# BrianPugh/tamp

Measured on AMD Instinct MI355X. Metric: input MB/s, 4KiB-chunk batch compress window=10 (bit-exact vs C ref), higher is better.
Workload: dtype u8

## Files before the change

### tamp_amd/csrc/tamp_common.hpp

```cpp
#pragma once
#include <hip/hip_runtime.h>
#include <stdint.h>

namespace tamp_amd {

constexpr int kWave = 64;
constexpr uint32_t kRing = 16;
constexpr uint32_t kPendMax = 256;
constexpr uint32_t kRleMax = 241;
constexpr uint32_t kRleWindowMax = 8;
constexpr uint32_t kExtExtraMax = 120;
constexpr int kSymRle = 12, kSymExt = 13, kSymFlush = 14;

enum : int8_t {
    kOk = 0,
    kOutputFull = 1,
    kInputExhausted = 2,
    kError = -1,
    kExcessBits = -2,
    kInvalidConf = -3,
    kOob = -4,
    kBadArgument = -21,
};

constexpr uint32_t kMaxDecodeIn = (1u << 29) - 1;
constexpr uint32_t kMaxDecodeCall = 1u << 28;

constexpr uint8_t kCodeTab[15] = {0x00, 0x03, 0x08, 0x0b, 0x14, 0x24, 0x26, 0x2b, 0x4b, 0x54, 0x94, 0x95, 0xaa, 0x27, 0xab};
constexpr uint8_t kNbitsTab[15] = {2, 3, 5, 5, 6, 7, 7, 7, 8, 8, 9, 9, 9, 7, 9};
constexpr uint64_t pack_bytes(const uint8_t* v, int first, int count) {
    uint64_t r = 0;
    for (int i = 0; i < count; i++) r |= (uint64_t)v[first + i] << (8 * i);
    return r;
}
constexpr uint64_t pack_nibbles(const uint8_t* v, int count) {
    uint64_t r = 0;
    for (int i = 0; i < count; i++) r |= (uint64_t)v[i] << (4 * i);
    return r;
}
constexpr uint64_t kCodeLo = pack_bytes(kCodeTab, 0, 8), kCodeHi = pack_bytes(kCodeTab, 8, 7);
constexpr uint64_t kNbitsPacked = pack_nibbles(kNbitsTab, 15);
static_assert(kCodeLo == 0x2b2624140b080300ull && kCodeHi == 0x00ab27aa9594544bull && kNbitsPacked == 0x979998877765532ull,
              "packed prefix code");
__device__ __forceinline__ uint32_t tok_code(uint32_t i) {
    return (uint32_t)((i < 8 ? kCodeLo >> (8 * i) : kCodeHi >> (8 * (i - 8))) & 0xFF);
}
__device__ __forceinline__ uint32_t tok_nbits(uint32_t i) { return (uint32_t)(kNbitsPacked >> (4 * i)) & 15; }

__host__ __device__ constexpr uint32_t align_up(uint32_t x, uint32_t a) { return (x + a - 1) & ~(a - 1); }

constexpr uint32_t kPackedMaxWbits = 14;
constexpr uint32_t max_code_nbits() {
    uint32_t m = 0;
    for (int i = 0; i < 15; i++) m = kNbitsTab[i] > m ? kNbitsTab[i] : m;
    return m;
}
constexpr uint32_t max_u32(uint32_t a, uint32_t b) { return a > b ? a : b; }
constexpr uint32_t kMaxTokenBits =
    max_u32(max_u32(1 + 8, max_code_nbits() + 15),
            max_u32(kNbitsTab[kSymRle] + max_code_nbits() - 1 + 4, kNbitsTab[kSymExt] + max_code_nbits() - 1 + 3 + kPackedMaxWbits));
static_assert(kMaxTokenBits <= 32, "a token is placed as one 32-bit value: at most two words of the bit buffer");

__host__ __device__ __forceinline__ void token_words(uint32_t v, uint32_t nb, uint32_t bitpos, uint32_t* wi, uint32_t* w_hi,
                                                     uint32_t* w_lo) {
    const uint32_t ph = bitpos & 31u;
    const uint64_t x = (uint64_t)v << (64u - ph - nb);
    *wi = bitpos >> 5;
    *w_hi = __builtin_bswap32((uint32_t)(x >> 32));
    *w_lo = __builtin_bswap32((uint32_t)x);
}

constexpr uint32_t kDictOffAlign = 16;
__host__ __device__ constexpr bool dict_off_aligned(uint64_t off) { return (off & (kDictOffAlign - 1)) == 0; }
__host__ __device__ constexpr bool dict_off_in_bounds(uint64_t off, uint32_t W, uint64_t len) { return off <= len && W <= len - off; }

__host__ __device__ constexpr int min_pattern_size(int window, int literal) {
    return 2 + (window > 10 + 2 * (literal - 5));
}

struct __attribute__((packed, aligned(1))) LdsU128 { uint32_t x, y, z, w; };

__device__ __forceinline__ uint32_t lds_u32_unaligned(const uint8_t* base, uint32_t off) {
    const uint32_t* w = reinterpret_cast<const uint32_t*>(base + (off & ~3u));
    return __builtin_amdgcn_alignbyte(w[1], w[0], off & 3u);
}

#if defined(__HIP_DEVICE_COMPILE__) && !defined(__GFX9__)
#error "tamp_amd device code is written for gfx9-family wave64 targets (gfx950); its DPP scans have no gfx10+ form"
#endif
template <class Op>
__device__ __forceinline__ uint32_t wave_scan_incl(uint32_t x, uint32_t identity, Op op) {
    x = op(x, (uint32_t)__builtin_amdgcn_update_dpp((int)identity, (int)x, 0x111, 0xF, 0xF, false));
    x = op(x, (uint32_t)__builtin_amdgcn_update_dpp((int)identity, (int)x, 0x112, 0xF, 0xF, false));
    x = op(x, (uint32_t)__builtin_amdgcn_update_dpp((int)identity, (int)x, 0x114, 0xF, 0xF, false));
    x = op(x, (uint32_t)__builtin_amdgcn_update_dpp((int)identity, (int)x, 0x118, 0xF, 0xF, false));
    x = op(x, (uint32_t)__builtin_amdgcn_update_dpp((int)identity, (int)x, 0x142, 0xA, 0xF, false));
    x = op(x, (uint32_t)__builtin_amdgcn_update_dpp((int)identity, (int)x, 0x143, 0xC, 0xF, false));
    return x;
}
__device__ __forceinline__ uint32_t wave_scan_add(uint32_t x) {
    return wave_scan_incl(x, 0u, [](uint32_t a, uint32_t b) { return a + b; });
}
__device__ __forceinline__ uint32_t wave_scan_max(uint32_t x) {
    return wave_scan_incl(x, 0u, [](uint32_t a, uint32_t b) { return a > b ? a : b; });
}

__device__ __forceinline__ uint32_t wave_max_u32(uint32_t v) {
#pragma unroll
    for (int off = 32; off > 0; off >>= 1) {
        uint32_t o = (uint32_t)__shfl_xor((int)v, off);
        v = o > v ? o : v;
    }
    return v;
}

}
```

### tamp_amd/csrc/tamp_compress_kernel.hpp

```cpp
#pragma once
#include "tamp_common.hpp"

namespace tamp_amd {

constexpr uint32_t kHashBits = 11;
constexpr uint32_t kHashBuckets = 1u << kHashBits;
constexpr uint32_t kRemBits = 16 - kHashBits;
constexpr uint32_t kRunCap = 128;
constexpr int kPrioScan = 0, kPrioShort = 2, kPrioWalk = 3;
constexpr uint32_t kDeferMin = 24;
constexpr uint32_t kDeferred = 0x1Fu;
constexpr uint32_t kLongRun = 8;
constexpr uint32_t kSlowCap = 128;
constexpr uint32_t kHb1024 = 10;

struct CompressArgs {
    const uint8_t* in;
    const uint64_t* in_off;
    const uint32_t* in_len;
    uint8_t* out;
    const uint64_t* out_off;
    const uint32_t* out_cap;
    uint32_t* out_len;
    int8_t* status;
// ... 525 lines not shown
                    }
                }
                ext_count = len;
                ext_pos = idx;
                rd += len;
                return kStepOk;
            }
            put((tok_code(len - minp) << wbits) | idx, tok_nbits(len - minp) + wbits);
        }
        const uint32_t rd0 = rd;
        rd += len;
        append(len, wr + len == rd, [&](uint32_t i) { return uni(ebuf[W + rd0 + i]); });
        return kStepOk;
    }
};

constexpr uint32_t kWgPerCu = 8, kLeanPerCu = 6, kLazyPerCu = 5;
constexpr uint32_t kBrkShift = 0, kBrkMin = 512;
constexpr uint32_t kAlignMin = 256;
enum : uint32_t { kActDone = 1, kActRebase = 2, kActContinue = 3 };
enum : uint8_t { kSegResume = 1, kSegSave = 2, kSegFlushToken = 4, kSegPartial = 8 };
enum : uint32_t {
    kSlotWindowPos = 0,
    kSlotToken = 2,
    kSlotRle = 3,
    kSlotExtCount = 4,
    kSlotNbits = 5,
    kSlotExtPos = 6,
    kSlotParsed = 9,
    kSlotBits = 16,
};
constexpr uint32_t kSegStateExtra = 24;
enum : uint32_t { cAct = 0, cShift = 1, cP0 = 2, cPending = 3, cWp = 4, cNtok = 5, cExcess = 6, cBlk = 7, cWave = 8, cNruns = 12, cQuad = 13, cNext = 14, cCut = 15, cCutThr = 16 };

#ifdef TAMP_PROF
#define TAMP_PROF_ONLY(...) __VA_ARGS__
#define TAMP_DBG(bit) ((a.dbg & (bit)) != 0)
#define TAMP_REPEAT(bit) for (uint32_t _rep = 0; _rep < (TAMP_DBG(bit) ? 2u : 1u); _rep++)
#define TAMP_SECOND (_rep != 0)
#define TAMP_FINE(v) do { unsigned long long _n = __builtin_readcyclecounter(); v += _n - fc; fc = _n; } while (0)
#define TAMP_PROF_MARK(i)                                     \
    do {                                                      \
        __syncthreads();                                      \
        unsigned long long _n = __builtin_readcyclecounter(); \
        pt[i] += _n - pc;                                     \
        pc = _n;                                              \
        if (TAMP_DBG(8u << (i))) return;                      \
    } while (0)
#else
#define TAMP_PROF_ONLY(...)
#define TAMP_DBG(bit) false
#define TAMP_REPEAT(bit)
#define TAMP_SECOND false
#define TAMP_FINE(v) do { } while (0)
#define TAMP_PROF_MARK(i) do { } while (0)
#endif

template <class T>
__device__ __forceinline__ T* as_global(T* p) {
    return (T*)(__attribute__((address_space(1))) T*)reinterpret_cast<uintptr_t>(p);
}

enum : uint32_t { kFixNone = 0, kFixExt = 1, kFixV1 = 2 };
constexpr uint32_t kFixWbits = 10, kFixBlk = 1024, kFixLbits = 8, kFixThreads = 256;
constexpr CompressLds kLdsFixed(1u << kFixWbits, kFixBlk, true, false, true, kHb1024);
static_assert(kLdsFixed.total == 19616 && kLdsFixed.tokcap == 1376 && kLdsFixed.obuf_words == 516,
              "the fixed builds' LDS layout is the generic build's for window 2^10, block 1,024, 1,024 buckets");
template <bool FX>
__device__ __forceinline__ uint8_t* lds_base() {
    if constexpr (FX) {
        __shared__ __attribute__((aligned(16))) uint8_t smem_fx[kLdsFixed.total];
        return smem_fx;
    } else {
        extern __shared__ __attribute__((aligned(16))) uint8_t smem[];
        return smem;
    }
}
template <bool PACKED, bool LAZY, bool RUNS, uint32_t WSCAN, uint32_t HB, bool LOOP, bool BLOCKM, uint32_t FIX, bool DICTS = false>
__device__ __forceinline__ void compress_streams(CompressArgs a_k) {
    static_assert(!DICTS || FIX == kFixNone, "table calls take the generic builds");
    static_assert(!BLOCKM || (LOOP && PACKED && !LAZY), "block mode: a persistent build of the default parse");
    constexpr bool FX = FIX != kFixNone;
    constexpr bool kFoldSort = FX, kOrTail = FX;
    static_assert(!FX || (PACKED && !LAZY && RUNS && WSCAN == (1u << kFixWbits) && HB == kHb1024 && LOOP && !BLOCKM),
                  "fixed geometry: the run-aware persistent build of the 2^10 window");
    static_assert(HB >= 9 && HB <= 11, "entry payload: 16 - HB bigram bits + 8 bits of the third byte + the rest of the fourth");
    constexpr uint32_t kRem = 16 - HB, kBuckets = 1u << HB;
    constexpr bool kEntV2 = PACKED && !LAZY;
    constexpr uint32_t kPB = WSCAN == 1024 ? 12u : 16u, kLB = 32u - kRem - kPB;
    static_assert(!kEntV2 || kLB >= 9, "the third byte and at least one bit of the fourth");
    static_assert(!(RUNS && LAZY), "the run list serves the default parse only");
    uint8_t* const smem = lds_base<FX>();
    typedef __attribute__((address_space(3))) volatile uint32_t LdsWord;
    constexpr uint32_t kNoClaim = 0xFFFFFFFFu;
    LdsWord* const claim = (LdsWord*)smem;
    if constexpr (LOOP) {
        if (threadIdx.x == 0) {
            const uint32_t nx = atomicAdd(a_k.work_counter, a_k.claim);
            claim[2] = nx, claim[0] = nx + 1, claim[1] = nx + a_k.claim, claim[3] = kNoClaim;
        }
        __syncthreads();
    }
    typedef const __attribute__((address_space(4))) uint32_t* KernArgs;
    struct ArgWords { uint32_t w[sizeof(CompressArgs) / 4]; };
    static_assert(sizeof(ArgWords) == sizeof(CompressArgs), "whole dwords");
    KernArgs ap = (KernArgs)__builtin_amdgcn_kernarg_segment_ptr();
    uint32_t wave_k = Walk::uni(threadIdx.x >> 6);
    for (;;) {
        ArgWords aw;
        if constexpr (LOOP) {
            asm volatile("" : "+s"(ap));
#pragma unroll
            for (uint32_t i = 0; i < (DICTS ? (uint32_t)(sizeof(CompressArgs) / 4) : kPlainArgWords); i++) aw.w[i] = ap[i];
        }
        CompressArgs a_l = __builtin_bit_cast(CompressArgs, aw);
        if constexpr (LOOP) {
            a_l.in = as_global(a_l.in), a_l.in_off = as_global(a_l.in_off), a_l.in_len = as_global(a_l.in_len);
            a_l.out = as_global(a_l.out), a_l.out_off = as_global(a_l.out_off), a_l.out_cap = as_global(a_l.out_cap);
            a_l.out_len = as_global(a_l.out_len), a_l.status = as_global(a_l.status), a_l.dict = as_global(a_l.dict);
            a_l.state = as_global(a_l.state), a_l.work_counter = as_global(a_l.work_counter), a_l.prof = as_global(a_l.prof);
            a_l.blk_table = as_global(a_l.blk_table), a_l.blk_info = as_global(a_l.blk_info);
            a_l.blk_len = as_global(a_l.blk_len), a_l.blk_idx = as_global(a_l.blk_idx);
            if constexpr (DICTS) a_l.dict_off = as_global(a_l.dict_off);
        }
        const CompressArgs& a = LOOP ? a_l : a_k;
        const uint32_t a_wbits = FX ? kFixWbits : a.wbits, a_blk = FX ? kFixBlk : a.blk;
        const uint32_t W = 1u << a_wbits, mask = W - 1;
        constexpr bool lazy = LAZY;
        const CompressLds L = FX ? kLdsFixed : CompressLds(W, a_blk, PACKED, lazy, RUNS, HB == 9 ? kHashBits : HB);
        uint8_t* const ebuf = smem + L.ebuf;
        uint16_t* const cnt16 = reinterpret_cast<uint16_t*>(smem + L.cnt);
        uint32_t* const cntw = reinterpret_cast<uint32_t*>(smem + L.cnt);
        uint32_t* const ent = reinterpret_cast<uint32_t*>(smem + L.ent);
        uint16_t* const ent16 = reinterpret_cast<uint16_t*>(smem + L.ent);
        uint16_t* const toklist = reinterpret_cast<uint16_t*>(smem + L.ent);
        uint16_t* const jump16 = reinterpret_cast<uint16_t*>(smem + L.ent + L.jump);
        uint8_t* const count8 = smem + L.ent + L.count;
        uint32_t* const jc32 = reinterpret_cast<uint32_t*>(smem + L.ent + L.jump);
        uint8_t* const vstep = smem + L.ent + L.vstep;
        uint32_t* const stok = reinterpret_cast<uint32_t*>(smem + L.cnt);
        uint8_t* const xcnt = smem + L.cnt + kSlowCap * 8;
        uint8_t* const blen = smem + L.blen;
        uint16_t* const bidx = reinterpret_cast<uint16_t*>(smem + L.bidx);
        uint8_t* const blen2 = smem + L.blen2;
        uint16_t* const bidx2 = reinterpret_cast<uint16_t*>(smem + L.bidx2);
        uint32_t* const obuf = reinterpret_cast<uint32_t*>(smem + L.obuf);
        uint16_t* const qstart = reinterpret_cast<uint16_t*>(smem + L.obuf + 16);
        uint16_t* const sorted = reinterpret_cast<uint16_t*>(smem + L.cnt);
        typedef __attribute__((address_space(3))) volatile uint32_t LdsCtl;
        LdsCtl* const ctl = (LdsCtl*)(smem + L.ctl);
        uint32_t* const bins = reinterpret_cast<uint32_t*>(smem + L.ctl + 80);
        uint8_t* const codetab = smem + L.ctl + 80 + 256;
        constexpr uint32_t kDictBadByte = 15;
        uint32_t* const runs = reinterpret_cast<uint32_t*>(smem + L.runs);
        uint32_t* const runsx = reinterpret_cast<uint32_t*>(smem + L.runsx);
        uint32_t* const rxset = reinterpret_cast<uint32_t*>(smem + L.rxset);
        uint32_t* const rbits = reinterpret_cast<uint32_t*>(smem + L.rbits);

        uint32_t tid_l = threadIdx.x;
        if constexpr (LOOP) {
            uint32_t lane_l;
            asm volatile("v_mbcnt_lo_u32_b32 %0, -1, 0\n\tv_mbcnt_hi_u32_b32 %0, -1, %0" : "=v"(lane_l));
            asm volatile("" : "+s"(wave_k));
            tid_l = (wave_k << 6) | lane_l;
        }
        const uint32_t tid_k = tid_l, nt = FX ? kFixThreads : blockDim.x;
        const uint32_t nt_log2 = nt == 256 ? 8u : 6u;
        uint32_t tid = tid_k;
        int lane = tid & (kWave - 1);
        uint32_t wave = tid >> 6;
        const uint32_t wbits = a_wbits, lbits = FX ? kFixLbits : a.lbits;
        const uint32_t minp = (uint32_t)min_pattern_size((int)a_wbits, (int)lbits);
        const bool ext = FX ? FIX == kFixExt : a.extended != 0;
        const uint32_t maxp = ext ? minp + 11 + kExtExtraMax : minp + 13;
#ifdef TAMP_POISON_LDS
        {
            __syncthreads();
            const uint32_t seed = (uint32_t)__builtin_readcyclecounter() | 1u;
            for (uint32_t k = 4 + tid_k; k < L.total / 4; k += nt)
                reinterpret_cast<uint32_t*>(smem)[k] = (TAMP_POISON_LDS) ? (k + 1) * 2654435761u * seed : 0xFFFFFFFFu;
            __syncthreads();
        }
#endif
        if (tid_k < 15) codetab[tid_k] = (uint8_t)tok_code(tid_k);
        if (RUNS && tid_k == 0) ctl[cQuad] = 0;

        uint32_t s;
        if constexpr (LOOP) {
            s = Walk::uni(claim[2]);
            if (s >= a.n_streams) break;
        } else {
            s = blockIdx.x + a.first_stream;
        }
        const uint32_t si = BLOCKM ? 0u : s;
        const uint8_t* const in = a.in + uni_u64(a.in_off[si]);
        const uint8_t* sdict = a.dict;
        bool dict_ok = true;
        if constexpr (DICTS) {
            const uint64_t off = uni_u64(a.dict_off[si]);
            dict_ok = dict_off_aligned(off) && dict_off_in_bounds(off, W, a.dict_len);
            sdict += dict_ok ? off : 0;
        }
        const uint32_t n = dict_ok ? Walk::uni(a.in_len[si]) : 0u;
        uint8_t* const gout = a.out + uni_u64(a.out_off[si]);
        const uint32_t cap = dict_ok ? Walk::uni(a.out_cap[si]) : 0u;
        const uint32_t bpos = BLOCKM ? s * a_blk : 0u;
        unsigned long long binfo = 0;
        if constexpr (BLOCKM) {
            if (a.block_pass == 3) binfo = uni_u64(a.blk_info[s]);
        }

        const uint32_t seg_flags = FX ? 0u : a.seg_flags;
        uint8_t* const st_io = (!FX && a.state) ? a.state + (size_t)s * (W + kSegStateExtra) : nullptr;
        const bool partial = (seg_flags & kSegPartial) != 0;
        uint32_t wp0 = 0;
        if constexpr (BLOCKM) {
            wp0 = bpos & mask;
            for (uint32_t k = tid; k < W; k += nt) ebuf[k] = (bpos + k >= W) ? in[bpos + k - W] : sdict[(bpos + k) & mask];
        } else
        if (st_io && (seg_flags & kSegResume)) {
            wp0 = (uint32_t)st_io[W + kSlotWindowPos] | ((uint32_t)st_io[W + kSlotWindowPos + 1] << 8);
            for (uint32_t k = tid; k < W; k += nt) ebuf[k] = st_io[(wp0 + k) & mask];
        } else if (DICTS && !dict_ok) {
        } else if (FX || (reinterpret_cast<uintptr_t>(sdict) & 3) == 0) {
            for (uint32_t k = tid * 4; k < W; k += nt * 4)
                *reinterpret_cast<uint32_t*>(ebuf + k) = *reinterpret_cast<const uint32_t*>(sdict + k);
        } else {
            for (uint32_t k = tid; k < W; k += nt) ebuf[k] = sdict[k];
        }
        uint32_t c_rle = 0, c_ext = 0, c_extpos = 0, c_nbits = 0, c_bits = 0;
        if (st_io && (seg_flags & kSegResume)) {
            c_rle = Walk::uni(st_io[W + kSlotRle]), c_ext = Walk::uni(st_io[W + kSlotExtCount]);
            c_nbits = Walk::uni(st_io[W + kSlotNbits]) & 31u;
            c_extpos = Walk::uni((uint32_t)st_io[W + kSlotExtPos] | ((uint32_t)st_io[W + kSlotExtPos + 1] << 8));
            c_bits = Walk::uni((uint32_t)st_io[W + kSlotBits] | ((uint32_t)st_io[W + kSlotBits + 1] << 8) |
                               ((uint32_t)st_io[W + kSlotBits + 2] << 16) | ((uint32_t)st_io[W + kSlotBits + 3] << 24));
        }
        const uint32_t nlead = FX ? 1u : a.nlead;
        const uint32_t word0 = (BLOCKM && s != 0) ? 0u : (nlead ? (uint32_t)a.lead << 16 : (c_nbits ? c_bits & (0xFFFFFFFFu << (32 - c_nbits)) : 0u));
        for (uint32_t k = tid; k < L.obuf_words; k += nt) obuf[k] = k == 0 ? __builtin_bswap32(word0) : 0;

        Walk wk;
        wk.ebuf = ebuf, wk.blen = blen, wk.bidx = bidx, wk.toklist = toklist, wk.stok = stok;
        wk.W = W, wk.mask = mask, wk.wbits = wbits, wk.lbits = lbits, wk.minp = minp, wk.ext = ext;
        wk.wp_e = wp0, wk.wr = 0, wk.rd = 0, wk.nvalid = 0;
        wk.rle_count = c_rle, wk.ext_count = c_ext, wk.ext_pos = c_extpos, wk.rd = c_rle + c_ext, wk.partial = partial;
        wk.ext_resolved = false, wk.ntok = 0, wk.ns = 0, wk.lane = lane;
        wk.ctlw = (Walk::CtlWord*)ctl, wk.coop = nt == 256;
        wk.lazy = lazy, wk.lazy_valid = false, wk.lazy_idx = 0, wk.lazy_len = 0, wk.blen2 = blen2, wk.bidx2 = bidx2;
        if (tid_k == 0) ctl[cCutThr] = (FIX == kFixV1) ? 0u : a.cut_run;
        if (DICTS && !BLOCKM && tid_k == 0) codetab[kDictBadByte] = dict_ok ? 0 : 1;
        uint32_t w_p0 = bpos;

        uint32_t carry = BLOCKM ? ((uint32_t)(binfo >> 4) & 31u) : (nlead ? 8u * nlead : c_nbits);
        uint32_t gpos = 0;
        uint32_t e_p0 = bpos, e_pending = c_rle + c_ext, e_wp = wp0;
        bool need_match = true;
        bool piece_done = false;
        uint32_t cur_blk = a_blk;
        TAMP_PROF_ONLY(unsigned long long pt[16] = {}, pc = __builtin_readcyclecounter();)
        for (;;) {
            asm volatile("" : "+v"(tid));
            lane = (int)(tid & (kWave - 1)), wave = tid >> 6, wk.lane = lane;
            const uint32_t left = n - e_p0;
            uint32_t nvalid = left < cur_blk ? left : cur_blk;
            if (ext && !LAZY) {
                const uint32_t k0 = W - e_wp;
                if (k0 >= kAlignMin && k0 < nvalid) nvalid = k0;
            }
            const uint32_t nplan = nvalid;
            if (!need_match) nvalid = Walk::uni(ctl[cCut]);
            uint32_t nv = LAZY ? 2 * nvalid : nvalid;
            const uint8_t* const steps = LAZY ? vstep : blen;
            if (need_match) {
                __builtin_amdgcn_s_setprio(kPrioShort);
                const uint32_t room = cur_blk + kRing + kPendMax;
                const uint32_t nload = left < room ? left : room;
                TAMP_REPEAT(0x10000u) {
                    const uint8_t* src = in + e_p0;
                    const uint32_t nfill = align_up(nload + 20, 4);
                    const uint32_t nw = nload >> 2;
                    for (uint32_t k = tid; k < nw; k += nt) {
                        uint32_t v;
                        __builtin_memcpy(&v, src + 4 * k, 4);
                        reinterpret_cast<uint32_t*>(ebuf + W)[k] = v;
                    }
                    for (uint32_t k = (nw << 2) + tid; k < nfill; k += nt) ebuf[W + k] = k < nload ? src[k] : 0;
                }
                for (uint32_t k = tid; k < kBuckets / 2; k += nt) cntw[k] = 0;
                if (tid == 0) ctl[cCut] = 0xFFFFFFFFu;
                __syncthreads();
                TAMP_PROF_MARK(0);
                TAMP_PROF_ONLY(pt[12] += 1, pt[13] += nvalid;)

                bool have_tables = false;
                if constexpr (BLOCKM) {
                    have_tables = a.block_pass == 3 && a.blk_len != nullptr;
                    if (have_tables) {
                        const uint8_t* const gl = a.blk_len + bpos;
                        const uint16_t* const gi = a.blk_idx + bpos;
                        for (uint32_t k = tid * 4; k < nvalid; k += nt * 4) {
                            *reinterpret_cast<uint32_t*>(blen + k) = *reinterpret_cast<const uint32_t*>(gl + k);
                            *reinterpret_cast<uint2*>(bidx + k) = *reinterpret_cast<const uint2*>(gi + k);
                        }
                        __syncthreads();
                        for (uint32_t k = nvalid + tid; k < nvalid + 128 && k < a_blk + 128; k += nt) blen[k] = 0x80;
                        __syncthreads();
                    }
                }
                if (!have_tables) {
#ifdef TAMP_PROF
                uint32_t index_reps = TAMP_DBG(0x20000u) ? 2u : 1u;
            index_again:
#endif
                asm volatile("" : "+v"(tid));
                lane = (int)(tid & (kWave - 1)), wave = tid >> 6, wk.lane = lane;
                const uint32_t NE0 = nvalid ? W + nvalid : 0;
                const uint32_t cut_run = (FIX == kFixV1) ? 0u : Walk::uni(ctl[cCutThr]);
                for (uint32_t c4 = tid * 4; c4 < NE0; c4 += nt * 4) {
                    const uint32_t d0 = *reinterpret_cast<const uint32_t*>(ebuf + c4);
                    const uint32_t d1 = *reinterpret_cast<const uint32_t*>(ebuf + c4 + 4);
                    if (d0 == (d0 & 0xFFu) * 0x01010101u) {
                        if constexpr (RUNS) ctl[cQuad] = 1;
                        if (cut_run && d1 == d0 && c4 >= W + e_pending + 4 && c4 + 4 * cut_run <= NE0) {
                            bool all = true;
                            for (uint32_t k = 2; k < cut_run; k++) all = all && *reinterpret_cast<const uint32_t*>(ebuf + c4 + 4 * k) == d0;
                            if (all) atomicMin((uint32_t*)&ctl[cCut], c4);
                        }
                    }
#pragma unroll
                    for (uint32_t j = 0; j < 4; j++) {
                        if (c4 + j < NE0) {
                            const uint32_t h = mix16<HB>(__builtin_amdgcn_alignbyte(d1, d0, j) & 0xFFFFu) >> kRem;
                            atomicAdd(&cntw[h >> 1], 1u << ((h & 1) * 16));
                            if (c4 >= W) qstart[c4 + j - W] = (uint16_t)h;
                        }
                    }
                }
                __syncthreads();
                {
                    const uint32_t cutc = Walk::uni(ctl[cCut]);
                    if (cutc < NE0) nvalid = cutc - W + 4, nv = LAZY ? 2 * nvalid : nvalid;
                }
                const uint32_t NE = nvalid ? W + nvalid : 0;
                for (uint32_t k = nvalid + tid; k < nvalid + 128 && k < a_blk + 128; k += nt) blen[k] = 0x80;
                uint32_t nruns = 0;
                if constexpr (RUNS) {
                    if (Walk::uni(ctl[cQuad])) {
                        for (uint32_t k = tid; k < (W + a_blk + 96) / 32; k += nt) rbits[k] = 0;
                        if (tid == 0) ctl[cNruns] = 0;
                        if (tid < 8) rxset[tid] = 0;
                        __syncthreads();
                        if (tid == 0) ctl[cQuad] = 0;
                        const uint32_t lim = NE + 16;
                        for (uint32_t c = tid; c < NE; c += nt) {
                            const uint32_t b4 = lds_u32_unaligned(ebuf, c), x = b4 & 0xFFu;
                            if (b4 == x * 0x01010101u && (c == 0 || ebuf[c - 1] != x)) {
                                uint32_t e = c + 4;
                                while ((e & 3u) && e < lim && ebuf[e] == x) e++;
                                if (!(e & 3u)) {
                                    while (e + 8 <= lim) {
                                        const uint32_t* wv = reinterpret_cast<const uint32_t*>(ebuf + e);
                                        const uint32_t v0 = wv[0], v1 = wv[1];
                                        if (v0 != b4 || v1 != b4) break;
                                        e += 8;
                                    }
                                    while (e < lim && ebuf[e] == x) e++;
                                }
                                if (e - c >= kLongRun) {
                                    const uint32_t slot = atomicAdd((uint32_t*)&ctl[cNruns], 1u);
                                    if (slot < kRunCap) {
                                        runs[slot] = c | (e << 16);
                                        runsx[slot] = x | ((lds_u32_unaligned(ebuf, e) & 0xFFFFu) << 8);
                                        atomicOr(&rxset[x >> 5], 1u << (x & 31u));
                                        for (uint32_t k = c + 1; k <= e - 4;) {
                                            const uint32_t hiw = min(e - 4, k | 31u);
                                            const uint32_t m = (0xFFFFFFFFu << (k & 31u)) & (0xFFFFFFFFu >> (31u - (hiw & 31u)));
                                            atomicOr(&rbits[k >> 5], m);
                                            k = hiw + 1;
                                        }
                                    }
                                }
                            }
                        }
                        __syncthreads();
                        nruns = min(Walk::uni(ctl[cNruns]), kRunCap);
                    }
                }
                {
                    const uint32_t per = kBuckets >> nt_log2;
                    uint32_t sum = 0;
                    for (uint32_t k = 0; k < per; k++) sum += cnt16[tid * per + k];
                    const uint32_t incl = wave_scan_add(sum);
                    if (lane == kWave - 1) ctl[cWave + wave] = incl;
                    __syncthreads();
                    uint32_t run = incl - sum;
                    for (uint32_t w2 = 0; w2 < wave; w2++) run += ctl[cWave + w2];
                    for (uint32_t k = 0; k < per; k++) {
                        uint32_t v = cnt16[tid * per + k];
                        cnt16[tid * per + k] = (uint16_t)run;
                        run += v;
                    }
                }
                __syncthreads();
                if (tid < nvalid) qstart[tid] = cnt16[qstart[tid]];
                if (kFoldSort && tid < 64) bins[tid] = 0;
                __syncthreads();
                for (uint32_t t0 = 0; t0 < NE; t0 += nt) {
                    const uint32_t c = t0 + tid;
                    uint32_t h = 0;
                    if (c < NE) {
                        const uint32_t b4 = lds_u32_unaligned(ebuf, c);
                        const uint32_t mx = mix16<HB>(b4 & 0xFFFFu);
                        h = mx >> kRem;
                        const uint32_t sh = (h & 1) * 16;
                        bool keep = true;
                        if constexpr (RUNS) { if (nruns) keep = !((rbits[c >> 5] >> (c & 31u)) & 1u); }
                        if (keep) {
                            const uint32_t old = atomicAdd(&cntw[h >> 1], 1u << sh);
                            if (kEntV2)
                                ent[(old >> sh) & 0xFFFFu] = ((mx & ((1u << kRem) - 1)) << (kPB + kLB)) | (c << kLB) | ((b4 >> 16) & ((1u << kLB) - 1));
                            else if (PACKED)
                                ent[(old >> sh) & 0xFFFFu] = c | entry_payload<kRem>(b4, mx);
                            else
                                ent16[(old >> sh) & 0xFFFFu] = (uint16_t)c;
                        }
                    }
                    __syncthreads();
                    if constexpr (!kFoldSort) {
                        if (c < NE && c >= W) bidx[c - W] = cnt16[h];
                    } else if (c < NE && c >= W) {
                        const uint32_t top = cnt16[h];
                        bidx[c - W] = (uint16_t)top;
                        if (c - W >= e_pending) {
                            const uint32_t Lq = min(top - (uint32_t)qstart[c - W], 63u);
                            atomicAdd(&bins[63 - Lq], 1u);
                            blen[c - W] = (uint8_t)Lq;
                        }
                    }
                    const uint32_t q2 = t0 + nt + tid;
                    if (q2 < nvalid) qstart[q2] = cnt16[qstart[q2]];
                    __syncthreads();
                }
                if (!kFoldSort && tid < 64) bins[tid] = 0;
                if (tid == 0) ctl[cCut] = nvalid;
                if constexpr (!kFoldSort) {
                    __syncthreads();
                    for (uint32_t q = e_pending + tid; q < nvalid; q += nt) {
                        const uint32_t Lq = min((uint32_t)bidx[q] - (uint32_t)qstart[q], 63u);
                        atomicAdd(&bins[63 - Lq], 1u);
                    }
                    __syncthreads();
                }
                if (wave == 0) {
                    const uint32_t v = bins[lane];
                    const uint32_t incl = wave_scan_add(v);
                    bins[lane] = incl - v;
                }
                __syncthreads();
                for (uint32_t q = e_pending + tid; q < nvalid; q += nt) {
                    const uint32_t Lq = kFoldSort ? (uint32_t)blen[q] : min((uint32_t)bidx[q] - (uint32_t)qstart[q], 63u);
                    sorted[atomicAdd(&bins[63 - Lq], 1u)] = (uint16_t)q;
                }
                __syncthreads();
#ifdef TAMP_PROF
                if (--index_reps) {
                    for (uint32_t k = tid; k < kBuckets / 2; k += nt) cntw[k] = 0;
                    if (tid == 0) ctl[cCut] = 0xFFFFFFFFu;
                    __syncthreads();
                    goto index_again;
                }
#endif
                TAMP_PROF_MARK(1);

                __builtin_amdgcn_s_setprio(kPrioScan);
                asm volatile("" : "+v"(tid));
                lane = (int)(tid & (kWave - 1)), wave = tid >> 6, wk.lane = lane;
                const uint32_t nq = nvalid - e_pending;
                TAMP_PROF_ONLY(unsigned long long f0 = 0, f1 = 0, f2 = 0, f3 = 0, niter = 0, fc = __builtin_readcyclecounter();)
                for (uint32_t j = tid; j < nq; j += nt) {
                    const uint32_t q = sorted[j];
                    const uint32_t leftq = n - (e_p0 + q);
                    const uint32_t R = leftq < kRing ? leftq : kRing;
                    uint32_t key = 0;
                    uint32_t wrapbest = 0, n16 = 0;
                    bool sole_ext = false;
                    uint32_t keyB = 0, wrapmaskB = 0, cap_lenB = 0;
                    if (lazy && q >= 1) {
                        const uint32_t leftp = n - (e_p0 + q - 1);
                        const uint32_t Rb = (leftp < kRing ? leftp : kRing) - 1;
                        cap_lenB = Rb >= minp ? (Rb < maxp ? Rb : maxp) : 0;
                    }
                    uint32_t P[4];
#pragma unroll
                    for (int jj = 0; jj < 4; jj++) P[jj] = lds_u32_unaligned(ebuf, W + q + 4 * jj);
                    const uint32_t rep = (P[0] & 0xFFu) * 0x01010101u;
                    bool in_run = false;
                    const uint32_t prevb = ebuf[W + q - 1];
                    if (ext && !lazy && (P[0] & 0xFFFFu) == prevb * 0x0101u) {
                        const uint32_t x0 = P[0] ^ rep, x1 = (P[1] ^ rep) & 0x00FFFFFFu;
                        const uint32_t r = x0 ? (uint32_t)__builtin_ctz(x0) >> 3 : (x1 ? 4 + ((uint32_t)__builtin_ctz(x1) >> 3) : 7u);
                        in_run = r >= 7 || r >= R;
                        if (!in_run && r >= 2 && (kFoldSort ? (uint32_t)blen[q] : (uint32_t)bidx[q] - (uint32_t)qstart[q]) >= kDeferMin) in_run = true, key = kDeferred << 16;
                    }
                    if (R >= minp && !in_run) {
                        const uint32_t cap_len = R < maxp ? R : maxp;
                        const uint32_t pk = entry_payload<kRem>(P[0], mix16<HB>(P[0] & 0xFFFFu));
                        const uint32_t chi = q + W - 2;
                        const uint32_t s_hi = bidx[q];
                        uint32_t sl = qstart[q], wrapmask = 0;
                        uint32_t e_next = PACKED ? ent[sl] : (uint32_t)ent16[sl];
                        TAMP_FINE(f0);
                        if constexpr (kEntV2) {
                            const uint32_t Ws = WSCAN ? WSCAN : W;
                            const uint32_t pkx = ((mix16<HB>(P[0] & 0xFFFFu) & ((1u << kRem) - 1)) << (kPB + kLB)) | ((P[0] >> 16) & ((1u << kLB) - 1));
                            const uint32_t qs = q << kLB;
                            const uint32_t nb = ~(q + e_wp);
                            const uint32_t* pe = ent + sl;
                            const uint32_t* const pe_end = ent + s_hi;
                            TAMP_REPEAT(0x100u) {
                            TAMP_PROF_ONLY(if (TAMP_SECOND) n16 = 0, pe = ent + sl, e_next = *pe;)
                            while (pe < pe_end) {
                                TAMP_PROF_ONLY(niter++;)
                                const uint32_t e = e_next;
                                pe++;
                                e_next = *pe;
                                const uint32_t y = (e ^ pkx) - qs;
                                if (y < ((Ws - 1) << kLB)) {
                                    const uint32_t d = y >> kLB;
                                    const uint32_t low = y & ((1u << kLB) - 1);
                                    uint32_t len = (low & 0xFFu) ? 2u : 3u;
                                    if (low == 0) {
                                        len = prefix_len16<kOrTail>(ebuf, q + d, P);
                                        if (TAMP_DBG(0x1000000u)) {
                                            asm volatile("" ::: "memory");
                                            len = max(len, prefix_len16<kOrTail>(ebuf, q + d, P));
                                        }
                                    }
                                    if (d + len >= Ws) {
                                        wrapmask |= 1u << (Ws - d);
                                    } else {
                                        if constexpr (RUNS) n16 += len >> 4;
                                        const uint32_t lim_i = ((nb - d) & (Ws - 1)) + 1;
                                        key = max(key, (min(len, min(cap_len, lim_i)) << 16) | lim_i);
                                    }
                                }
                            }
                            }
                        } else if constexpr (!LAZY) {
                            const uint32_t Ws = WSCAN ? WSCAN : W;
                            TAMP_PROF_ONLY(const uint32_t sl0 = sl;)
                            TAMP_REPEAT(0x100u) {
                            TAMP_PROF_ONLY(if (TAMP_SECOND) n16 = 0, sl = sl0, e_next = PACKED ? ent[sl] : (uint32_t)ent16[sl];)
                            while (sl < s_hi) {
                                TAMP_PROF_ONLY(niter++;)
                                const uint32_t e = e_next;
                                sl++;
                                e_next = PACKED ? ent[sl] : (uint32_t)ent16[sl];
                                const uint32_t x = PACKED ? (e ^ pk) >> 16 : 0u;
                                const uint32_t c = e & 0xFFFFu;
                                const uint32_t d = c - q;
                                const uint32_t i = (e + e_wp) & (Ws - 1);
                                if (d <= Ws - 2 && (x & ((1u << kRem) - 1)) == 0) {
                                    const uint32_t t = Ws - d;
                                    uint32_t len = (x & (0xFFu << kRem)) ? 2u : 3u;
                                    if ((x >> kRem) == 0) {
                                        len = prefix_len16(ebuf, c, P);
                                        if (TAMP_DBG(0x1000000u)) {
                                            asm volatile("" ::: "memory");
                                            len = max(len, prefix_len16(ebuf, c, P));
                                        }
                                    }
                                    if (t < 16 && len >= t) {
                                        wrapmask |= 1u << t;
                                    } else {
                                        if constexpr (RUNS) n16 += len >> 4;
                                        const uint32_t lim_i = Ws - i;
                                        key = max(key, (min(len, min(cap_len, lim_i)) << 16) | lim_i);
// ... 29 lines not shown
                            }
                            if (okB) {
                                if (t <= 16) {
                                    wrapmaskB |= 1u << (t - 1);
                                } else {
                                    const uint32_t l2 = min(len, min(cap_lenB, W - i));
                                    const uint32_t k = (l2 << 16) | (0xFFFFu - i);
                                    if (l2 >= 2 && k > keyB) keyB = k;
                                }
                            }
                        }
                        if (prevb == (P[0] & 0xFFu) && ebuf[q] == ((P[0] >> 8) & 0xFFu)) wrapmask |= 2u;
                        TAMP_PROF_ONLY(const uint32_t wrapmask0 = wrapmask;)
                        TAMP_REPEAT(0x200u) {
                        TAMP_PROF_ONLY(wrapmask = wrapmask0;)
                        while (wrapmask) {
                            const uint32_t t = (uint32_t)__builtin_ctz(wrapmask);
                            wrapmask &= wrapmask - 1;
                            const uint32_t c = q + W - t;
                            const uint32_t i = (e_wp + c) & mask;
                            if (i == mask) continue;
                            const uint32_t lw = prefix_len_wrapped16(ebuf, c, t, W, P);
                            if constexpr (RUNS) wrapbest = max(wrapbest, lw);
                            const uint32_t len = min(lw, min(cap_len, W - i));
                            const uint32_t k = (len << 16) | (W - i);
                            if (len >= 2 && k > key) key = k;
                        }
                        }
                        if constexpr (RUNS) {
                            const uint32_t len0 = key >> 16;
                            if (ext && len0 > minp + 11 && !(nruns && P[0] == rep) && (len0 < 16 || (n16 == 1 && wrapbest < 16)))
                                sole_ext = true;
                        }
                    }
                    if (cap_lenB) {
                        {
                            const uint32_t c = q - 1, i = (e_wp + c) & mask;
                            if (i != mask) {
                                const uint32_t l2 = min(prefix_len16(ebuf, c, P), min(cap_lenB, W - i));
                                const uint32_t k = (l2 << 16) | (0xFFFFu - i);
                                if (l2 >= 2 && k > keyB) keyB = k;
                            }
                        }
                        if (ebuf[q + W - 2] == (P[0] & 0xFFu)) wrapmaskB |= 2u;
                        while (wrapmaskB) {
                            const uint32_t t = (uint32_t)__builtin_ctz(wrapmaskB);
                            wrapmaskB &= wrapmaskB - 1;
                            const uint32_t c = q - 1 + W - t;
                            const uint32_t i = (e_wp + c) & mask;
                            if (i == mask) continue;
                            const uint32_t l2 = min(prefix_len_wrapped16(ebuf, c, t, W, P), min(cap_lenB, W - i));
                            const uint32_t k = (l2 << 16) | (0xFFFFu - i);
                            if (l2 >= 2 && k > keyB) keyB = k;
                        }
                    }
                    if (lazy && q >= 1) {
                        blen2[q - 1] = (uint8_t)(keyB >> 16);
                        bidx2[q - 1] = (uint16_t)(0xFFFFu - (keyB & 0xFFFFu));
                    }
                    const uint32_t len = key >> 16;
                    bool slow = false;
                    if (ext) {
                        const uint32_t prev = prevb, b0 = P[0] & 0xFFu, b1 = (P[0] >> 8) & 0xFFu;
                        slow = (prev == b0 && (b1 == b0 || R == 1)) || (!lazy && len > minp + 11);
                    }
                    if (partial && leftq < kRing) slow = true;
                    blen[q] = (uint8_t)(len | (slow ? 0x80u : 0u) | (RUNS && sole_ext ? 0x40u : 0u));
                    bidx[q] = (uint16_t)(W - (key & 0xFFFFu));
                    TAMP_FINE(f2);
                }
                if constexpr (RUNS) {
                    if (nruns)
                    TAMP_REPEAT(0x2000000u) {
                        for (uint32_t j = tid; j < nq; j += nt) {
                            const uint32_t q = sorted[j];
                            const uint32_t b01 = lds_u32_unaligned(ebuf, W + q);
                            const uint32_t x = b01 & 0xFFu;
                            if (((b01 >> 8) & 0xFFu) != x) continue;
                            if (!((rxset[x >> 5] >> (x & 31u)) & 1u)) continue;
                            const uint32_t leftq = n - (e_p0 + q);
                            const uint32_t R = leftq < kRing ? leftq : kRing;
                            if (R < minp) continue;
                            uint32_t P[4];
#pragma unroll
                            for (int jj = 0; jj < 4; jj++) P[jj] = lds_u32_unaligned(ebuf, W + q + 4 * jj);
                            const uint32_t rep = x * 0x01010101u;
                            uint32_t rq = 16;
#pragma unroll
                            for (int jj = 3; jj >= 0; jj--) {
                                const uint32_t xx = P[jj] ^ rep;
                                if (xx) rq = 4u * (uint32_t)jj + ((uint32_t)__builtin_ctz(xx) >> 3);
                            }
                            if (ext && ebuf[W + q - 1] == x && (min(rq, 7u) >= 7u || rq >= R)) continue;
                            const uint32_t cap_len = R < maxp ? R : maxp;
                            const uint32_t sv = blen[q];
                            if ((sv & 0x1Fu) == kDeferred) continue;
                            uint32_t key = (sv & 0x1Fu) ? (((sv & 0x1Fu) << 16) | (W - (uint32_t)bidx[q])) : 0u;
                            const uint32_t key0 = key;
                            bool hit16 = false;
                            {
                                const uint32_t wz = q + W - 16, sh = wz & 31u;
                                uint32_t rb16 = rbits[wz >> 5] >> sh;
                                if (sh > 16) rb16 |= rbits[(wz >> 5) + 1] << (32u - sh);
                                uint32_t wrapmask = (__builtin_bitreverse32(rb16) >> 15) & 0xFFFCu;
                                while (wrapmask) {
                                    const uint32_t t = (uint32_t)__builtin_ctz(wrapmask);
                                    wrapmask &= wrapmask - 1;
                                    const uint32_t c = q + W - t;
                                    if (ebuf[c] != x) continue;
                                    const uint32_t i = (e_wp + c) & mask;
                                    if (i == mask) continue;
                                    const uint32_t lw = prefix_len_wrapped16(ebuf, c, t, W, P);
                                    hit16 = hit16 || lw >= 16;
                                    const uint32_t len = min(lw, min(cap_len, W - i));
                                    const uint32_t k = (len << 16) | (W - i);
                                    if (len >= 2 && k > key) key = k;
                                }
                            }
                            const uint32_t cz = q + ((0u - e_wp - q) & mask);
                            const uint32_t qhi = q + W - 16;
                            const uint32_t pb2 = lds_u32_unaligned(ebuf, W + q + (rq < 16 ? rq : 0u)) & 0xFFFFu;
#pragma unroll 1
                            for (uint32_t k = 0; k < nruns; k++) {
                                const uint32_t rv = Walk::uni(runs[k]), rx = Walk::uni(runsx[k]);
                                const uint32_t ra = rv & 0xFFFFu, rb = rv >> 16;
                                const uint32_t lo = max(ra + 1, q), hi = min(rb - 4, qhi);
                                if ((rx & 0xFFu) != x || lo > hi) continue;
                                const int32_t cs = (int32_t)rb - (int32_t)rq;
                                const bool cz_in = cz >= lo && cz <= hi;
                                {
                                    const int32_t hiA = min((int32_t)hi, cs - 1);
                                    if ((int32_t)lo <= hiA) {
                                        const uint32_t c = cz_in && (int32_t)cz <= hiA ? cz : lo;
                                        const uint32_t lim_i = W - ((c + e_wp) & mask);
                                        key = max(key, (min(rq, min(cap_len, lim_i)) << 16) | lim_i);
                                    }
                                }
                                if (cs >= (int32_t)lo && cs <= (int32_t)hi) {
                                    const uint32_t x2 = (rx >> 8) ^ pb2;
                                    uint32_t len = rq;
                                    if (rq < 16 && !(x2 & 0xFFu)) len = (x2 >> 8) ? rq + 1 : prefix_len16<kOrTail>(ebuf, (uint32_t)cs, P);
                                    const uint32_t lim_i = W - (((uint32_t)cs + e_wp) & mask);
                                    key = max(key, (min(len, min(cap_len, lim_i)) << 16) | lim_i);
                                }
                                {
                                    const int32_t c1 = max((int32_t)lo, cs + 1);
                                    if (c1 <= (int32_t)hi) {
                                        const uint32_t lim_i = W - (((uint32_t)c1 + e_wp) & mask);
                                        key = max(key, (min(rb - (uint32_t)c1, min(cap_len, lim_i)) << 16) | lim_i);
                                        if (cz_in && (int32_t)cz > c1) key = max(key, (min(rb - cz, cap_len) << 16) | W);
                                    }
                                }
                            }
                            if (key != key0 || (hit16 && (sv & 0x40u))) {
                                const uint32_t len = key >> 16;
                                const bool slow = (sv & 0x80u) || (ext && len > minp + 11);
                                blen[q] = (uint8_t)(len | (slow ? 0x80u : 0u));
                                bidx[q] = (uint16_t)(W - (key & 0xFFFFu));
                            }
                        }
                    }
                }
                __syncthreads();
                __builtin_amdgcn_s_setprio(kPrioShort);
                TAMP_FINE(f3);
                TAMP_PROF_ONLY(pt[6] += f0, pt[7] += f1, pt[8] += f2, pt[10] += niter;)
                if constexpr (RUNS && PACKED) {
                    if (ext && (kSlowCap * 8 + a_blk) <= (HB == 9 ? kHashBuckets : kBuckets) * 2) {
                        const uint32_t max_ext = minp + 11 + kExtExtraMax;
                        TAMP_REPEAT(0x4000000u)
                        for (uint32_t q = e_pending + tid; q < nvalid; q += nt) {
                            const bool dry = TAMP_DBG(0x4000000u) && !TAMP_SECOND;
                            const uint32_t sv = blen[q];
                            if (!(sv & 0x80u)) continue;
                            const uint32_t len = sv & 0x1Fu;
                            if (len == kDeferred) continue;
                            const uint32_t leftq = n - (e_p0 + q);
                            if (partial && leftq < kRing) continue;
                            const uint32_t wpq = (e_wp + q) & mask;
                            const uint32_t b4 = lds_u32_unaligned(ebuf, W + q - 1);
                            const uint32_t prev = b4 & 0xFFu, b0 = (b4 >> 8) & 0xFFu, b1 = (b4 >> 16) & 0xFFu;
                            if (prev == b0) {
                                if (b1 != b0 || leftq < 2) continue;
                                const uint32_t rep = b0 * 0x01010101u;
                                const uint32_t x0 = lds_u32_unaligned(ebuf, W + q + 2) ^ rep, x1 = lds_u32_unaligned(ebuf, W + q + 6) ^ rep;
                                const uint32_t r = 2u + (x0 ? (uint32_t)__builtin_ctz(x0) >> 3 : 4u + (x1 ? (uint32_t)__builtin_ctz(x1) >> 3 : 4u));
                                if (r > kRleWindowMax || r >= leftq || wpq + r > W) continue;
                                if (r <= 6 && len > r) {
                                    if (len <= minp + 11 && !dry) blen[q] = (uint8_t)len;
                                    continue;
                                }
                                if (!dry) blen[q] = (uint8_t)(0x20u | 1u), xcnt[q] = (uint8_t)r;
                                continue;
                            }
                            if (!(sv & 0x40u)) continue;
                            const uint32_t idx = bidx[q];
                            const uint32_t off = (idx - wpq) & mask, t0 = W - off;
                            const uint32_t lim = min(min(W - idx, max_ext), min(leftq, t0));
                            uint32_t m = 0;
                            while (m < lim) {
                                const uint32_t x = lds_u32_unaligned(ebuf, q + off + m) ^ lds_u32_unaligned(ebuf, W + q + m);
                                if (x) {
                                    m += (uint32_t)__builtin_ctz(x) >> 3;
                                    break;
                                }
                                m += 4;
                            }
                            const uint32_t cnt = min(m, lim);
                            if (cnt >= t0 || cnt < len || wpq + cnt > W) continue;
                            if (partial && leftq <= cnt + kRing) continue;
                            if (!dry) blen[q] = (uint8_t)(0x20u | len), xcnt[q] = (uint8_t)cnt;
                        }
                    }
                    __syncthreads();
                }
                }
                for (uint32_t k = 4 + tid; k < 4 + a_blk / 2 && k < L.obuf_words; k += nt) obuf[k] = 0;
                if constexpr (LAZY) {
                    for (uint32_t v = tid; v < nv + 128 && v < 2 * a_blk + 128; v += nt) {
                        uint32_t out = 0x80u;
                        const uint32_t pp = v >> 1, s1 = v & 1u;
                        if (v < nv && pp + 1 < nvalid && !(s1 && pp == 0)) {
                            const uint32_t sva = blen[pp];
                            const uint32_t len = s1 ? (uint32_t)blen2[pp - 1] : (sva & 0x1Fu);
                            if (!(sva & 0x80u) && !(ext && len > minp + 11)) {
                                const uint32_t leftp = n - (e_p0 + pp);
                                const uint32_t R = leftp < kRing ? leftp : kRing;
                                bool defer = false;
                                if (len >= minp && len <= 8 && R > len + 2) {
                                    const uint32_t nlen = blen2[pp], nidx = bidx2[pp];
                                    const uint32_t wpos = (e_wp + pp) & mask;
                                    defer = nlen > len && (wpos < nidx || wpos >= nidx + nlen);
                                }
                                out = defer ? 3u - s1 : 2u * (len >= minp ? len : 1u) - s1;
                            }
                        }
                        vstep[v] = (uint8_t)out;
                    }
                    __syncthreads();
                }
                TAMP_REPEAT(0x40000u)
                for (uint32_t b = wave * 64; b < nv; b += (nt >> 6) * 64) {
                    const uint32_t sv = steps[b + lane];
                    const bool slowp = (sv & 0x80u) != 0;
                    uint32_t stepv = LAZY ? (sv & 0x7Fu) : (sv >= minp ? (sv & 0x1Fu) : 1u);
                    if constexpr (RUNS && PACKED) {
                        if (sv & 0x20u) stepv = xcnt[b + lane];
                        if (b + lane < nv) xcnt[b + lane] = (uint8_t)stepv;
                    }
                    constexpr uint32_t kCnt = (0xFFu << 10) | (BLOCKM ? 0xFFF80000u : 0u);
                    const uint32_t tgt = (uint32_t)lane + stepv;
                    const bool endp = slowp || tgt >= 64u;
                    uint32_t own = 1u << 10;
                    if constexpr (BLOCKM) {
                        const uint32_t lenv = sv & 0x1Fu;
                        own |= (lenv >= minp ? tok_nbits(lenv - minp) + wbits : lbits + 1u) << 19;
                    }
                    uint32_t st = endp ? ((uint32_t)lane << 2) : ((tgt << 2) | own);
                    const uint32_t endv = slowp ? ((uint32_t)lane << 2) : ((tgt << 2) | own);
#pragma unroll
                    for (int r = 0; r < 6; r++) {
                        const uint32_t o2 = (uint32_t)__builtin_amdgcn_ds_bpermute((int)(st & 0x3FFu), (int)st);
                        st = o2 + (st & kCnt);
                    }
                    {
                        const uint32_t e = (uint32_t)__builtin_amdgcn_ds_bpermute((int)(st & 0x3FFu), (int)endv);
                        st = e + (st & kCnt);
                    }
                    if constexpr (BLOCKM) {
                        if (a.block_pass == 1 && b + lane < nv) toklist[b + lane] = (uint16_t)(st >> 19);
                    }
                    st = ((st & 0x3FFu) >> 2) | (((st >> 10) & 0xFFu) << 8);
                    if (b + lane < nv) {
                        if constexpr (LAZY) {
                            jump16[b + lane] = (uint16_t)(b + (st & 0xFFu));
                            count8[b + lane] = (uint8_t)((st >> 8) & 0xFFu);
                        } else {
                            jc32[b + lane] = (b + (st & 0xFFu)) | (((st >> 8) & 0xFFu) << 16);
                        }
                    }
                }
                __syncthreads();
                TAMP_PROF_MARK(2);
            }
            if constexpr (BLOCKM) {
                if (a.block_pass == 1) {
                    if (tid < 16) {
                        uint32_t pos = tid, bits = 0;
                        bool ok = tid < 15;
                        while (ok && pos < nvalid) {
                            const uint32_t jc = jc32[pos], j = jc & 0xFFFFu;
                            if (j == pos) { ok = false; break; }
                            bits += toklist[pos];
                            pos = j;
                        }
                        a.blk_table[(size_t)s * 16 + tid] = ok ? ((pos - nvalid) | (bits << 4)) : 0xFFFFFFFFu;
                    }
                    if (a.blk_len) {
                        uint8_t* const gl = a.blk_len + bpos;
// ... 466 lines not shown
```

Measured before the change: 59220.

## Specialize fixed-geometry build: shared LDS pattern loads, quad histogram, constant-trip init loops

For the fixed 2^10-window build, it loads pattern bytes with N+1 aligned LDS words plus alignbyte, so consecutive unaligned reads share one set of loads instead of reloading overlapping words. The bigram histogram pass hashes four positions at once from two words and stores four hashes as one uint2. Zero-fill and sentinel loops become single per-thread uint2 stores sized by compile-time constants. This aims to cut LDS traffic and loop overhead in the hot per-block setup. The cost is extra code paths only valid for the fixed geometry, guarded by static asserts.

```diff
diff --git a/tamp_amd/csrc/tamp_common.hpp b/tamp_amd/csrc/tamp_common.hpp
--- a/tamp_amd/csrc/tamp_common.hpp
+++ b/tamp_amd/csrc/tamp_common.hpp
@@ -85,6 +85,17 @@
     return __builtin_amdgcn_alignbyte(w[1], w[0], off & 3u);
 }
 
+template <int N>
+__device__ __forceinline__ void lds_bytes_unaligned(const uint8_t* base, uint32_t off, uint32_t (&P)[N]) {
+    const uint32_t* w = reinterpret_cast<const uint32_t*>(base + (off & ~3u));
+    const uint32_t sh = off & 3u;
+    uint32_t d[N + 1];
+#pragma unroll
+    for (int j = 0; j <= N; j++) d[j] = w[j];
+#pragma unroll
+    for (int j = 0; j < N; j++) P[j] = __builtin_amdgcn_alignbyte(d[j + 1], d[j], sh);
+}
+
 #if defined(__HIP_DEVICE_COMPILE__) && !defined(__GFX9__)
 #error "tamp_amd device code is written for gfx9-family wave64 targets (gfx950); its DPP scans have no gfx10+ form"
 #endif
diff --git a/tamp_amd/csrc/tamp_compress_kernel.hpp b/tamp_amd/csrc/tamp_compress_kernel.hpp
--- a/tamp_amd/csrc/tamp_compress_kernel.hpp
+++ b/tamp_amd/csrc/tamp_compress_kernel.hpp
@@ -631,6 +631,7 @@
     static_assert(!BLOCKM || (LOOP && PACKED && !LAZY), "block mode: a persistent build of the default parse");
     constexpr bool FX = FIX != kFixNone;
     constexpr bool kFoldSort = FX, kOrTail = FX;
+    constexpr bool kPat16 = FX, kQuadHist = FX, kConstLoops = FX;
     static_assert(!FX || (PACKED && !LAZY && RUNS && WSCAN == (1u << kFixWbits) && HB == kHb1024 && LOOP && !BLOCKM),
                   "fixed geometry: the run-aware persistent build of the 2^10 window");
     static_assert(HB >= 9 && HB <= 11, "entry payload: 16 - HB bigram bits + 8 bits of the third byte + the rest of the fourth");
@@ -787,6 +788,12 @@
         }
         const uint32_t nlead = FX ? 1u : a.nlead;
         const uint32_t word0 = (BLOCKM && s != 0) ? 0u : (nlead ? (uint32_t)a.lead << 16 : (c_nbits ? c_bits & (0xFFFFFFFFu << (32 - c_nbits)) : 0u));
+        if constexpr (kConstLoops) {
+            static_assert(kLdsFixed.obuf_words % 2 == 0 && kLdsFixed.obuf_words / 2 >= kFixThreads && kLdsFixed.obuf_words / 2 <= 2 * kFixThreads, "pairs of words: one per thread and a guarded tail");
+            uint2* const obuf2 = reinterpret_cast<uint2*>(obuf);
+            obuf2[tid] = make_uint2(tid == 0 ? __builtin_bswap32(word0) : 0u, 0u);
+            if (tid < kLdsFixed.obuf_words / 2 - kFixThreads) obuf2[kFixThreads + tid] = make_uint2(0u, 0u);
+        } else
         for (uint32_t k = tid; k < L.obuf_words; k += nt) obuf[k] = k == 0 ? __builtin_bswap32(word0) : 0;
 
         Walk wk;
@@ -836,6 +843,10 @@
                     }
                     for (uint32_t k = (nw << 2) + tid; k < nfill; k += nt) ebuf[W + k] = k < nload ? src[k] : 0;
                 }
+                if constexpr (kConstLoops) {
+                    static_assert(!kConstLoops || kBuckets / 2 == 2 * kFixThreads, "the cursor words: one pair per thread");
+                    reinterpret_cast<uint2*>(cntw)[tid] = make_uint2(0u, 0u);
+                } else
                 for (uint32_t k = tid; k < kBuckets / 2; k += nt) cntw[k] = 0;
                 if (tid == 0) ctl[cCut] = 0xFFFFFFFFu;
                 __syncthreads();
@@ -877,6 +888,16 @@
                             if (all) atomicMin((uint32_t*)&ctl[cCut], c4);
                         }
                     }
+                    if (kQuadHist && c4 + 4 <= NE0) {
+                        uint32_t hq[4];
+                        hq[0] = mix16<HB>(d0 & 0xFFFFu) >> kRem;
+#pragma unroll
+                        for (uint32_t j = 1; j < 4; j++) hq[j] = mix16<HB>(__builtin_amdgcn_alignbyte(d1, d0, j) & 0xFFFFu) >> kRem;
+#pragma unroll
+                        for (uint32_t j = 0; j < 4; j++) atomicAdd(&cntw[hq[j] >> 1], 1u << ((hq[j] & 1) * 16));
+                        if (c4 >= W) *reinterpret_cast<uint2*>(qstart + (c4 - W)) = make_uint2(hq[0] | (hq[1] << 16), hq[2] | (hq[3] << 16));
+                        continue;
+                    }
 #pragma unroll
                     for (uint32_t j = 0; j < 4; j++) {
                         if (c4 + j < NE0) {
@@ -892,10 +913,18 @@
                     if (cutc < NE0) nvalid = cutc - W + 4, nv = LAZY ? 2 * nvalid : nvalid;
                 }
                 const uint32_t NE = nvalid ? W + nvalid : 0;
+                if constexpr (kConstLoops) {
+                    static_assert(kFixThreads >= 128, "one sentinel per thread");
+                    if (tid < 128) blen[nvalid + tid] = 0x80;
+                } else
                 for (uint32_t k = nvalid + tid; k < nvalid + 128 && k < a_blk + 128; k += nt) blen[k] = 0x80;
                 uint32_t nruns = 0;
                 if constexpr (RUNS) {
                     if (Walk::uni(ctl[cQuad])) {
+                        if constexpr (kConstLoops) {
+                            static_assert(((1u << kFixWbits) + kFixBlk + 96) / 32 <= kFixThreads, "the bitmap: a word per thread at most");
+                            if (tid < ((1u << kFixWbits) + kFixBlk + 96) / 32) rbits[tid] = 0;
+                        } else
                         for (uint32_t k = tid; k < (W + a_blk + 96) / 32; k += nt) rbits[k] = 0;
                         if (tid == 0) ctl[cNruns] = 0;
                         if (tid < 8) rxset[tid] = 0;
@@ -1041,8 +1070,12 @@
                         cap_lenB = Rb >= minp ? (Rb < maxp ? Rb : maxp) : 0;
                     }
                     uint32_t P[4];
+                    if constexpr (kPat16) {
+                        lds_bytes_unaligned(ebuf, W + q, P);
+                    } else {
 #pragma unroll
-                    for (int jj = 0; jj < 4; jj++) P[jj] = lds_u32_unaligned(ebuf, W + q + 4 * jj);
+                        for (int jj = 0; jj < 4; jj++) P[jj] = lds_u32_unaligned(ebuf, W + q + 4 * jj);
+                    }
                     const uint32_t rep = (P[0] & 0xFFu) * 0x01010101u;
                     bool in_run = false;
                     const uint32_t prevb = ebuf[W + q - 1];
@@ -1238,8 +1271,12 @@
                             const uint32_t R = leftq < kRing ? leftq : kRing;
                             if (R < minp) continue;
                             uint32_t P[4];
+                            if constexpr (kPat16) {
+                                lds_bytes_unaligned(ebuf, W + q, P);
+                            } else {
 #pragma unroll
-                            for (int jj = 0; jj < 4; jj++) P[jj] = lds_u32_unaligned(ebuf, W + q + 4 * jj);
+                                for (int jj = 0; jj < 4; jj++) P[jj] = lds_u32_unaligned(ebuf, W + q + 4 * jj);
+                            }
                             const uint32_t rep = x * 0x01010101u;
                             uint32_t rq = 16;
 #pragma unroll
@@ -1334,12 +1371,15 @@
                             const uint32_t leftq = n - (e_p0 + q);
                             if (partial && leftq < kRing) continue;
                             const uint32_t wpq = (e_wp + q) & mask;
-                            const uint32_t b4 = lds_u32_unaligned(ebuf, W + q - 1);
+                            uint32_t A[3] = {0, 0, 0};
+                            if constexpr (kPat16) lds_bytes_unaligned(ebuf, W + q - 1, A);
+                            const uint32_t b4 = kPat16 ? A[0] : lds_u32_unaligned(ebuf, W + q - 1);
                             const uint32_t prev = b4 & 0xFFu, b0 = (b4 >> 8) & 0xFFu, b1 = (b4 >> 16) & 0xFFu;
                             if (prev == b0) {
                                 if (b1 != b0 || leftq < 2) continue;
                                 const uint32_t rep = b0 * 0x01010101u;
-                                const uint32_t x0 = lds_u32_unaligned(ebuf, W + q + 2) ^ rep, x1 = lds_u32_unaligned(ebuf, W + q + 6) ^ rep;
+                                const uint32_t x0 = (kPat16 ? __builtin_amdgcn_alignbyte(A[1], A[0], 3) : lds_u32_unaligned(ebuf, W + q + 2)) ^ rep;
+                                const uint32_t x1 = (kPat16 ? __builtin_amdgcn_alignbyte(A[2], A[1], 3) : lds_u32_unaligned(ebuf, W + q + 6)) ^ rep;
                                 const uint32_t r = 2u + (x0 ? (uint32_t)__builtin_ctz(x0) >> 3 : 4u + (x1 ? (uint32_t)__builtin_ctz(x1) >> 3 : 4u));
                                 if (r > kRleWindowMax || r >= leftq || wpq + r > W) continue;
                                 if (r <= 6 && len > r) {
@@ -1371,6 +1411,10 @@
                     __syncthreads();
                 }
                 }
+                if constexpr (kConstLoops) {
+                    static_assert(kFixBlk / 2 == 2 * kFixThreads && 4 + kFixBlk / 2 <= kLdsFixed.obuf_words, "the scan starts: one pair of words per thread");
+                    reinterpret_cast<uint2*>(obuf + 4)[tid] = make_uint2(0u, 0u);
+                } else
                 for (uint32_t k = 4 + tid; k < 4 + a_blk / 2 && k < L.obuf_words; k += nt) obuf[k] = 0;
                 if constexpr (LAZY) {
                     for (uint32_t v = tid; v < nv + 128 && v < 2 * a_blk + 128; v += nt) {
```

After: 60700 (median of 6 runs). 2.5% higher.
